# MarinerQ/npf_GWwaveform

Measured on AMD Instinct MI355X. Metric: waveform target-points/sec (train step), higher is better.
Workload: dtype f32 (every contraction of the step: fp32 operands as three exact bf16 terms, six v_mfma_f32_16x16x32_bf16 per product group, f32 accumulation -- f32 results, DESIGN.md 3.1 / 3.2; the 1-4-wide first / last layers: f32 FMAs); 1 GPU; BASELINE config 2: AttnCNP scaledot, r=256, 4-layer xy-encoder/decoder, 256 context / 1024 target points, 256 tasks per GPU (256 global), fp32 train step (fwd+loss+bwd+allreduce+Adam); tasks_per_gpu=256, global_tasks=256, context_points=256, target_points=1024, r_dim=256, n_params=799588, parallelism=dp1, hip_graph=True

## Files before the change

include/npf_hip.h:

```cpp
#ifndef NPF_HIP_H
#define NPF_HIP_H

#include <stdint.h>

#ifdef __cplusplus
extern "C" {
#endif

#define NPF_OK 0
#define NPF_EINVAL (-1)
#define NPF_ELAUNCH (-2)

#define NPF_MAX_OPS 40
#define NPF_MAX_FEATURES 512

enum npf_opcode {
  NPF_OP_END = 0,
  NPF_OP_LOAD_PT = 1,
  NPF_OP_STORE_PT = 2,
  NPF_OP_LOAD_ROWS = 3,
  NPF_OP_STORE_ROWS = 4,
  NPF_OP_LINEAR = 5,
  NPF_OP_SOFTMAX = 6,
  NPF_OP_ADD_PT = 7,
// ... 120 lines not shown
int npf_unpack_pt(const float *pt, int32_t n_tasks, int32_t pts_per_task, int32_t F_valid, float *rows,
                  void *stream);
int npf_transpose(const float *src, int32_t rows, int32_t cols, float *dst, void *stream);
int npf_split_heads(const float *src, int32_t n_tasks, int32_t pts_per_task, int32_t F, int32_t n_heads, float *dst,
                    void *stream);
int npf_merge_heads(const float *src, int32_t n_tasks, int32_t pts_per_task, int32_t F, int32_t n_heads, float *dst,
                    void *stream);

int npf_mha_fwd(const float *q, const float *k, const float *v, int32_t n_tasks, int32_t n_heads, int32_t n_keys,
                int32_t n_queries, int32_t F, float *out, float *lse, void *stream);
int npf_mha_bwd(const float *q, const float *k, const float *v, const float *out, const float *d_out, const float *lse,
                int32_t n_tasks, int32_t n_heads, int32_t n_keys, int32_t n_queries, int32_t F, float *d_q, float *d_k, float *d_v,
                void *stream);

int npf_add_layernorm_fwd(const float *a, const float *b, const float *gamma, const float *beta, float eps, int32_t n_tasks,
                          int32_t pts_per_task, int32_t F, float *y, float *stats, void *stream);
int npf_add_layernorm_bwd(const float *a, const float *b, const float *gamma, const float *stats, const float *dy, int32_t n_tasks,
                          int32_t pts_per_task, int32_t F, float *dx, float *partials, void *stream);

int npf_gather_points(const float *x, const float *y, const int64_t *idx, int32_t n_tasks, int32_t n_points,
                      int32_t n_sel, int32_t x_dim, int32_t y_dim, float *out_x, float *out_y, void *stream);

int npf_cast_bf16_weights(const float *src, int32_t n_rows, int32_t n_cols, int32_t ld, int32_t transposed, void *dst,
                          void *stream);

typedef struct npf_wprep_job {
  const float *src;
  void *dst;
  int32_t n_rows, n_cols, ld, kind;
} npf_wprep_job_t;
#define NPF_MAX_WPREP_JOBS 32
int npf_prepare_weights(const npf_wprep_job_t *jobs, int32_t n_jobs, void *stream);

#define NPF_X6_MAX_LAYERS 8
typedef struct {
  const void *w_img;
  const float *bias;
  const float *mask;
  float *store_in;
  float *store_out;
  const float *addend;
  unsigned long long *store_bits;
  const unsigned long long *mask_bits;
  int32_t relu;
  int32_t reserved;
} npf_x6_layer_t;
int npf_mlp_x6_run(const npf_x6_layer_t *layers, int32_t n_layers, const float *x, float *y, int32_t n_tasks,
                   int32_t tiles_per_task, void *stream);
int npf_mlp_x6_run_rows(const npf_x6_layer_t *layers, int32_t n_layers, const float *x, const float *in_rows, const float *in_w,
                        float *y, const float *out_w, const float *out_b, float *out_rows, int32_t n_tasks,
                        int32_t tiles_per_task, void *stream);

#define NPF_X6_MAX_OPS 12
typedef struct npf_x6_op {
  const float *in_pt;
  const float *in_rows;
  const float *in_w;
  const float *in_b;
  const float *pre_add;
  const float *mask;
  const unsigned long long *mask_bits;
  const float *sbwd_p;
  float *store_in;
  unsigned long long *store_in_bits;
  const void *w_img;
  int64_t w_task_stride;
  const float *bias;
  int64_t bias_task_stride;
  const float *addend;
  float *store_out;
  unsigned long long *store_bits;
  int32_t in_n;
  int32_t in_relu;
  int32_t relu;
  int32_t softmax_n;
  float softmax_scale;
  float sbwd_scale;
  int32_t reserved[2];
} npf_x6_op_t;
#define NPF_X6_IN_RM 1
#define NPF_X6_ADD_RM 2
#define NPF_X6_STORE_IN_F32 4
#define NPF_X6_STORE_OUT_F32 8
#define NPF_X6_DEFAULT_VARIANT 3
int npf_x6_run_ex(const npf_x6_op_t *ops, int32_t n_ops, const float *out_w, const float *out_b, float *out_rows,
                  int32_t n_tasks, int32_t tiles_per_task, int32_t pts_per_task, int32_t per_task, int32_t width,
                  int32_t variant, void *stream);
int npf_x6_run(const npf_x6_op_t *ops, int32_t n_ops, const float *out_w, const float *out_b, float *out_rows,
               int32_t n_tasks, int32_t tiles_per_task, int32_t per_task, int32_t width, void *stream);
int npf_x6_task_images(const float *src, int32_t n_tasks, int32_t pts, int32_t width, void *row_img, void *tr_img, void *stream);

int npf_b16_run(const npf_x6_op_t *ops, int32_t n_ops, const float *out_w, const float *out_b, float *out_rows, int32_t n_tasks,
                int32_t tiles_per_task, int32_t per_task, int32_t width, int32_t variant, void *stream);
int npf_b16_task_images(const float *src, int32_t n_tasks, int32_t pts, int32_t width, void *row_img, void *tr_img, void *stream);

int npf_masked_attn_fwd(const float *q, const float *k, const float *v, const int32_t *n_valid, int32_t n_tasks, int32_t n_keys,
                        int32_t n_queries, int32_t d, float scale, float *out, float *lse, void *stream);
int npf_masked_attn_bwd(const float *q, const float *k, const float *v, const int32_t *n_valid, const float *out, const float *d_out,
                        const float *lse, int32_t n_tasks, int32_t n_keys, int32_t n_queries, int32_t d, float scale, float *d_q,
                        float *d_k, float *d_v, void *stream);
int npf_masked_attn_fwd_nq(const float *q, const float *k, const float *v, const int32_t *n_valid, const int32_t *n_q_valid,
                           int32_t n_tasks, int32_t n_keys, int32_t n_queries, int32_t d, float scale, float *out, float *lse,
                           void *stream);
int npf_masked_attn_bwd_nq(const float *q, const float *k, const float *v, const int32_t *n_valid, const int32_t *n_q_valid,
                           const float *out, const float *d_out, const float *lse, int32_t n_tasks, int32_t n_keys, int32_t n_queries,
                           int32_t d, float scale, float *d_q, float *d_k, float *d_v, void *stream);
int npf_masked_attn_fwd_prefix(const float *q, const float *k_pre, const float *v_pre, const int32_t *n_prefix, const float *k_tail,
                               const float *v_tail, const int32_t *n_tail, const int32_t *n_q_valid, int32_t n_tasks,
                               int32_t n_prefix_tasks, int32_t c_pad, int32_t m_tail, int32_t n_queries, int32_t d, float scale,
                               float *out, void *stream);
int npf_masked_attn_fwd_loo(const float *q, const float *k, const float *v, const int32_t *n_valid, const int32_t *n_q_valid,
                            int32_t n_tasks, int32_t n_keys, int32_t n_queries, int32_t d, float scale, float *out, void *stream);
int npf_masked_mean_fwd(const float *R_pt, const int32_t *n_valid, int32_t n_tasks, int32_t pts_per_task, int32_t F, float *out,
                        void *stream);
int npf_masked_mean_bwd(const float *d_out, const int32_t *n_valid, int32_t n_tasks, int32_t pts_per_task, int32_t F, float *dR_pt,
                        int32_t accumulate, void *stream);
int npf_loo_mean(const float *R_pt, const int32_t *n_valid, int32_t n_tasks, int32_t pts_per_task, int32_t F, float *out,
                 void *stream);

#define NPF_APPEND_MAX_PAIRS 3
typedef struct npf_append_pair {
  const float *src;
  float *dst;
  int32_t F;
  int32_t reserved;
} npf_append_pair_t;
int npf_append_points(const npf_append_pair_t *pairs, int32_t n_pairs, int32_t *n_valid, const int32_t *n_new, int32_t n_tasks,
                      int32_t n_rows, int32_t capacity, void *stream);

int npf_version(void);

#ifdef __cplusplus
}
#endif
#endif
```

npf_gwwaveform_amd/csrc/x6_kernel.hip:

```cpp
#include "x6_args.hpp"


namespace npf {

template <int KF>
struct XpGeom {
  static constexpr int NB = KF / 16;
  static constexpr int KS = KF / 32;
  static constexpr int RowB = KF * 2;
  static constexpr int TermB = 16 * RowB;
  static constexpr int SlabB = 3 * TermB;
  static constexpr int Slots = 3;
  static constexpr int RPP = 1024 / RowB;
  static constexpr int PPT = 16 / RPP;
  static constexpr int NP = 3 * PPT / 4;
  static constexpr int BiasB = 2 * KF * 4;
};

__device__ __forceinline__ void xp_split(const f32x4& lo, const f32x4& hi, xp_u32x4& t0, xp_u32x4& t1, xp_u32x4& t2) {
#ifdef XP_NO_SPLIT
  t0 = __builtin_bit_cast(xp_u32x4, lo);
  t1 = __builtin_bit_cast(xp_u32x4, hi);
  t2 = t0 ^ t1;
  return;
#endif
  const float v[8] = {lo[0], lo[1], lo[2], lo[3], hi[0], hi[1], hi[2], hi[3]};
#pragma unroll
  for (int p = 0; p < 4; ++p) {
    const float a = v[2 * p], b = v[2 * p + 1];
    const unsigned h = xp_cvt_pk(a, b);
    const float ra = a - __builtin_bit_cast(float, h << 16), rb = b - __builtin_bit_cast(float, h & 0xffff0000u);
    const unsigned m = xp_cvt_pk(ra, rb);
    const float la = ra - __builtin_bit_cast(float, m << 16), lb = rb - __builtin_bit_cast(float, m & 0xffff0000u);
    t0[p] = h;
    t1[p] = m;
    t2[p] = xp_cvt_pk(la, lb);
  }
}

template <int KF, int NPG, int NW, int LA = 2>
__global__ __launch_bounds__(NW * 64, (NW == 4 && KF * NPG <= 256) ? 2 : 1) void x6_program_kernel(const XpArgs a) {
  using G = XpGeom<KF>;
  constexpr int NB = G::NB, KS = G::KS;
  constexpr int Slots = LA + 1;
  static_assert(LA >= 2 && LA <= 4 && LA <= NB, "slab look-ahead");
  constexpr int TPW = (NPG == 2 ? 4 : 2) * (NW / 4);
  constexpr int NPW = 3 * G::PPT / NW;
  static_assert(NPG == 1 || NPG == 2, "a wave owns half a tile or a whole one");
  static_assert((NW == 4 || NW == 8) && (3 * G::PPT) % NW == 0 && NPW <= KS, "pieces dealt evenly, one per k-step");
  __shared__ __attribute__((aligned(16))) char smem[Slots * G::SlabB + G::BiasB];
  const int tid = threadIdx.x, lane = tid & 63;
  const int wave = __builtin_amdgcn_readfirstlane(tid >> 6);
  const int p = lane & 15, g = lane >> 4;
  int bid = blockIdx.x;
  if (a.xcd_remap) bid = (bid & 7) * (int)(gridDim.x >> 3) + (bid >> 3);
  const int w_tile = NPG == 2 ? wave : (wave >> 1);
  const int half0 = NPG == 2 ? 0 : (wave & 1);
  int task, t_in;
  bool valid;
  if (a.wgs_per_task > 0) {
    task = bid / a.wgs_per_task;
    t_in = (bid - task * a.wgs_per_task) * TPW + w_tile;
    valid = t_in < a.tiles_per_task;
  } else {
    const long t = (long)bid * TPW + w_tile;
    valid = t < a.total_tiles;
    task = valid ? (int)(t / a.tiles_per_task) : 0;
    t_in = valid ? (int)(t - (long)task * a.tiles_per_task) : 0;
  }
#ifdef XP_NO_STORE
  valid = valid && a.n_ops > 1000;
#endif
  const long tile = valid ? (long)task * a.tiles_per_task + t_in : 0;
  if (a.wgs_per_task == 0) task = 0;
  const size_t tile_off = (size_t)tile * (KF * 32);
  const unsigned lane_b = (unsigned)(((16 * half0 + p) * 4 + g * 128) * 4);
  const size_t bits_off = ((size_t)tile * 2 + half0) * 64;
  const size_t row_off = (size_t)tile * 32 + 16 * half0;
  auto pt32 = [&](const float* base, int pg, int b) -> f32x4* {
    return (f32x4*)((char*)const_cast<float*>(base + tile_off + (size_t)(b * 512 + 64 * pg)) + lane_b);
  };
  auto rm32 = [&](const float* base, int pg, int b) -> const f32x4* {
    int pt = (valid ? t_in : 0) * 32 + 16 * (half0 + pg) + p;
    pt = pt < a.pts_per_task ? pt : a.pts_per_task - 1;
    const size_t tk = valid ? (size_t)(tile / a.tiles_per_task) : 0;
    return (const f32x4*)(base + (tk * a.pts_per_task + (size_t)pt) * KF + 4 * g + 16 * b);
  };

  constexpr int LPR = 64 / G::RPP;
  constexpr int NDL = G::PPT / NW > 0 ? G::PPT / NW : 1;
  unsigned dma_lane[NDL];
#pragma unroll
  for (int n = 0; n < NDL; ++n) {
    const int r0 = G::RPP * ((wave + NW * n) % G::PPT), row = r0 + lane / LPR, pos = lane % LPR;
    dma_lane[n] = (unsigned)((lane / LPR) * G::RowB + ((pos ^ (row & 15)) << 4));
  }
  const int n_slabs = a.n_mm * NB;
  auto dma_piece = [&](const char* img, int rows, char* slot, int n) {
#ifdef XP_NO_DMA
    return;
#endif
    const char* base = img + (size_t)rows * G::RowB;
    asm volatile("" : "+s"(base));
    const int q = wave + NW * n, term = q / G::PPT, r0 = G::RPP * (q % G::PPT);
    xp_dma16(base + (size_t)term * ((size_t)KF * KF * 2) + r0 * G::RowB + dma_lane[n % NDL], slot + term * G::TermB + r0 * G::RowB);
  };
  auto mm_base = [&](int j) { return a.mm_img[j] + (size_t)task * a.mm_stride[j]; };
  auto dma_slab = [&](int S, char* slot) {
    const char* img = mm_base(S / NB);
#pragma unroll
    for (int n = 0; n < NPW; ++n) dma_piece(img, (S % NB) * 16, slot, n);
  };
  const unsigned lds0 = (unsigned)(size_t)(__attribute__((address_space(3))) char*)smem;
  const unsigned lane_row = (unsigned)(p * G::RowB);
  float* bias_lds = (float*)(smem + Slots * G::SlabB);

#pragma unroll
  for (int i = 0; i < LA; ++i)
    if (n_slabs > i) dma_slab(i, smem + i * G::SlabB);
  int slot = 0, S0 = 0, jm = 0;
  f32x4 cur[NPG][NB];
#pragma unroll
  for (int pg = 0; pg < NPG; ++pg)
#pragma unroll
    for (int b = 0; b < NB; ++b) cur[pg][b] = f32x4{0.f, 0.f, 0.f, 0.f};

  for (int l = 0; l < a.n_ops; ++l) {
    const npf_x6_op_t& o = a.op[l];
    const int oflags = o.reserved[0];
#pragma unroll
    for (int pg = 0; pg < NPG; ++pg) {
      if (o.in_pt != nullptr) {
        if (oflags & NPF_X6_IN_RM) {
#pragma unroll
          for (int b = 0; b < NB; ++b) cur[pg][b] = *rm32(o.in_pt, pg, b);
        } else {
#pragma unroll
          for (int b = 0; b < NB; ++b) cur[pg][b] = *pt32(o.in_pt, pg, b);
        }
      }
      if (o.in_rows != nullptr) {
        const f32x4 r = ((const f32x4*)o.in_rows)[row_off + 16 * pg + p];
        const int nb_in = o.in_n >> 4;
#pragma unroll
        for (int b = 0; b < NB; ++b) {
          f32x4 v = {0.f, 0.f, 0.f, 0.f};
          if (b < nb_in) {
            const int f = 16 * b + 4 * g;
            if (o.in_b != nullptr) v = *(const f32x4*)(o.in_b + f);
#pragma unroll
            for (int n = 0; n < 4; ++n) {
              const f32x4 w = *(const f32x4*)(o.in_w + (size_t)n * o.in_n + f);
#pragma unroll
              for (int e = 0; e < 4; ++e) v[e] = fmaf(r[n], w[e], v[e]);
            }
            if (o.in_relu) {
#pragma unroll
              for (int e = 0; e < 4; ++e) v[e] = fmaxf(v[e], 0.f);
            }
          }
          cur[pg][b] = v;
        }
      }
      if (o.pre_add != nullptr) {
#pragma unroll
        for (int b = 0; b < NB; ++b) cur[pg][b] += *pt32(o.pre_add, pg, b);
      }
      if (o.mask != nullptr) {
#pragma unroll
        for (int b = 0; b < NB; ++b) {
          const f32x4 v = *pt32(o.mask, pg, b);
#pragma unroll
          for (int e = 0; e < 4; ++e) cur[pg][b][e] = v[e] > 0.f ? cur[pg][b][e] : 0.f;
        }
      }
      if constexpr (NB <= 16) {
        if (o.mask_bits != nullptr) {
          const unsigned long long w = o.mask_bits[bits_off + 64 * pg + lane];
          const int wl = (int)(unsigned)w, wh = (int)(unsigned)(w >> 32);
#pragma unroll
          for (int b = 0; b < NB; ++b)
#pragma unroll
            for (int e = 0; e < 4; ++e) {
              const int m = __builtin_amdgcn_sbfe(b < 8 ? wl : wh, 4 * (b & 7) + e, 1);
              const float x = cur[pg][b][e];
              cur[pg][b][e] = __int_as_float(__float_as_int(x) & m);
            }
        }
      }
      if constexpr (NB <= 16) if (o.sbwd_p != nullptr) {
        f32x4 P[NB];
        float dot = 0.f;
#pragma unroll
        for (int b = 0; b < NB; ++b) {
          P[b] = *pt32(o.sbwd_p, pg, b);
#pragma unroll
          for (int e = 0; e < 4; ++e) dot = fmaf(cur[pg][b][e], P[b][e], dot);
        }
        dot = xp_sum4(dot);
#pragma unroll
        for (int b = 0; b < NB; ++b)
#pragma unroll
          for (int e = 0; e < 4; ++e) cur[pg][b][e] = o.sbwd_scale * P[b][e] * (cur[pg][b][e] - dot);
      }
      if (o.store_in != nullptr && valid) {
#pragma unroll
        for (int b = 0; b < NB; ++b) __builtin_nontemporal_store(cur[pg][b], pt32(o.store_in, pg, b));
      }
      if constexpr (NB <= 16) {
        if (o.store_in_bits != nullptr && valid) {
          unsigned wlo = 0u, whi = 0u;
#pragma unroll
          for (int b = 0; b < NB; ++b)
#pragma unroll
            for (int e = 0; e < 4; ++e) (b < 8 ? wlo : whi) |= (unsigned)(cur[pg][b][e] > 0.f) << (4 * (b & 7) + e);
          o.store_in_bits[bits_off + 64 * pg + lane] = ((unsigned long long)whi << 32) | wlo;
        }
      }
    }
    if (o.w_img == nullptr) continue;

    for (int i = tid; i < KF; i += NW * 64)
      bias_lds[(jm & 1) * KF + i] = o.bias != nullptr ? o.bias[(size_t)task * o.bias_task_stride + i] : 0.f;
    xp_u32x4 tb[NPG][3][KS];
#pragma unroll
    for (int pg = 0; pg < NPG; ++pg)
#pragma unroll
      for (int st = 0; st < KS; ++st) xp_split(cur[pg][2 * st], cur[pg][2 * st + 1], tb[pg][0][st], tb[pg][1][st], tb[pg][2][st]);
    const bool has_add = o.addend != nullptr;
    if (has_add) {
#pragma unroll
      for (int pg = 0; pg < NPG; ++pg) {
        if (oflags & NPF_X6_ADD_RM) {
#pragma unroll
          for (int b = 0; b < NB; ++b) cur[pg][b] = *rm32(o.addend, pg, b);
        } else {
#pragma unroll
          for (int b = 0; b < NB; ++b) cur[pg][b] = *pt32(o.addend, pg, b);
        }
      }
    }
    const char* const img0 = mm_base(jm);
    const char* const img1 = mm_base(jm + 1 < a.n_mm ? jm + 1 : jm);
    const bool post = NB <= 16 && o.softmax_n > 0;
    const float* const out = (o.store_out != nullptr && valid && !post) ? o.store_out : nullptr;
    const unsigned bias_l = lds0 + Slots * G::SlabB + (jm & 1) * (KF * 4) + g * 16;
    const bool relu = o.relu != 0;
    unsigned pos_lo[NPG], pos_hi[NPG];
#pragma unroll
    for (int pg = 0; pg < NPG; ++pg) pos_lo[pg] = pos_hi[pg] = 0u;
#pragma unroll
    for (int s = 0; s < NB; ++s) {
      const int S = S0 + s;
      {
        const int rem = n_slabs - 1 - S;
#define XP_WAIT(N) asm volatile("s_waitcnt vmcnt(%0) lgkmcnt(0)\n\ts_barrier" ::"n"(N) : "memory")
        if (rem >= LA - 1) XP_WAIT((LA - 1) * NPW);
        else if (LA > 3 && rem == 2) XP_WAIT(2 * NPW);
        else if (LA > 2 && rem == 1) XP_WAIT(NPW);
        else XP_WAIT(0);
#undef XP_WAIT
      }
      const bool more = S + LA < n_slabs;
      char* const nslot = smem + ((slot + LA) % Slots) * G::SlabB;
      const unsigned sl = lds0 + slot * G::SlabB + lane_row;
      f32x4 acc[NPG], sm[NPG];
      xp_u32x4 fr[2][3];
#ifdef XP_NO_FRAG
      acc[0] = f32x4{0.f, 0.f, 0.f, 0.f};
      asm volatile("" : "=v"(fr[0][0]), "=v"(fr[0][1]), "=v"(fr[0][2]), "=v"(fr[1][0]), "=v"(fr[1][1]), "=v"(fr[1][2]));
#else
      asm volatile("ds_read_b128 %0, %4\n\tds_read_b128 %1, %5\n\tds_read_b128 %2, %5 offset:%6\n\tds_read_b128 %3, %5 offset:%7"
                   : "=&v"(acc[0]), "=&v"(fr[0][0]), "=&v"(fr[0][1]), "=&v"(fr[0][2])
                   : "v"(bias_l + 64 * s), "v"(sl + (((0 + g) ^ p) << 4)), "n"(G::TermB), "n"(2 * G::TermB));
#endif
#pragma unroll
      for (int st = 0; st < KS; ++st) {
        const int c = st & 1, n = c ^ 1;
        if (st < NPW && more) {
          asm volatile("s_waitcnt lgkmcnt(0)" ::: "memory");
          dma_piece(s + LA < NB ? img0 : img1, ((s + LA) % NB) * 16, nslot, st);
        }
#ifdef XP_NO_FRAG
        if (false) {
#else
        if (st + 1 < KS) {
#endif
          asm volatile("s_waitcnt lgkmcnt(0)\n\tds_read_b128 %0, %7\n\tds_read_b128 %1, %7 offset:%8\n\tds_read_b128 %2, %7 offset:%9"
                       : "=&v"(fr[n][0]), "=&v"(fr[n][1]), "=&v"(fr[n][2]), "+v"(fr[c][0]), "+v"(fr[c][1]), "+v"(fr[c][2]), "+v"(acc[0])
                       : "v"(sl + (((4 * (st + 1) + g) ^ p) << 4)), "n"(G::TermB), "n"(2 * G::TermB));
        } else {
          asm volatile("s_waitcnt lgkmcnt(0)" : "+v"(fr[c][0]), "+v"(fr[c][1]), "+v"(fr[c][2]), "+v"(acc[0]));
        }
        if (st == 0) {
#pragma unroll
          for (int pg = 0; pg < NPG; ++pg) {
            if (pg > 0) acc[pg] = acc[0];
            sm[pg] = f32x4{0.f, 0.f, 0.f, 0.f};
          }
        }
#ifdef XP_NO_MFMA
#define XPMM(A, B, C, PG) asm volatile("" : "+v"(C[PG]) : "v"(fr[c][A]), "v"(tb[PG][B][st]))
#else
#define XPMM(A, B, C, PG)                                                                                            \
  C[PG] = __builtin_amdgcn_mfma_f32_16x16x32_bf16(__builtin_bit_cast(xp_bf16x8, fr[c][A]),                           \
                                                  __builtin_bit_cast(xp_bf16x8, tb[PG][B][st]), C[PG], 0, 0, 0)
#endif
        if constexpr (NPG == 1) {
          XPMM(2, 0, sm, 0);
          XPMM(0, 0, acc, 0);
          XPMM(0, 2, sm, 0);
          XPMM(1, 0, acc, 0);
          XPMM(1, 1, sm, 0);
          XPMM(0, 1, acc, 0);
        } else {
          XPMM(2, 0, sm, 0);
          XPMM(2, 0, sm, 1);
          XPMM(0, 0, acc, 0);
          XPMM(0, 0, acc, 1);
          XPMM(0, 2, sm, 0);
          XPMM(0, 2, sm, 1);
          XPMM(1, 0, acc, 0);
          XPMM(1, 0, acc, 1);
          XPMM(1, 1, sm, 0);
          XPMM(1, 1, sm, 1);
          XPMM(0, 1, acc, 0);
          XPMM(0, 1, acc, 1);
        }
#undef XPMM
      }
#pragma unroll
      for (int pg = 0; pg < NPG; ++pg) {
        f32x4 r = acc[pg] + sm[pg];
        if (has_add) {
          asm volatile("" ::: "memory");
          r += cur[pg][s];
        }
        if (relu) {
#pragma unroll
          for (int e = 0; e < 4; ++e) {
            float x = r[e];
            asm("v_max_f32 %0, 0, %0" : "+v"(x));
            r[e] = x;
          }
        }
        cur[pg][s] = r;
        if (out != nullptr) __builtin_nontemporal_store(r, pt32(out, pg, s));
        if constexpr (NB <= 16) {
#pragma unroll
          for (int e = 0; e < 4; ++e) (s < 8 ? pos_lo[pg] : pos_hi[pg]) |= (unsigned)(r[e] > 0.f) << (4 * (s & 7) + e);
        }
      }
      slot = (slot + 1) % Slots;
    }
    S0 += NB;
    ++jm;
    if constexpr (NB <= 16) if (post) {
      const float sc = o.softmax_scale;
      const int n_valid = o.softmax_n;
#pragma unroll
      for (int pg = 0; pg < NPG; ++pg) {
        float mx = -INFINITY;
#pragma unroll
        for (int b = 0; b < NB; ++b)
#pragma unroll
          for (int e = 0; e < 4; ++e) {
            const bool ok = 16 * b + 4 * g + e < n_valid;
            cur[pg][b][e] = ok ? sc * cur[pg][b][e] : -INFINITY;
            mx = fmaxf(mx, cur[pg][b][e]);
          }
        mx = xp_max4(mx);
        float sum = 0.f;
#pragma unroll
        for (int b = 0; b < NB; ++b)
#pragma unroll
          for (int e = 0; e < 4; ++e) {
            cur[pg][b][e] = expf(cur[pg][b][e] - mx);
            sum += cur[pg][b][e];
          }
        sum = xp_sum4(sum);
        const float inv = 1.f / sum;
#pragma unroll
        for (int b = 0; b < NB; ++b)
#pragma unroll
          for (int e = 0; e < 4; ++e) cur[pg][b][e] *= inv;
        if (o.store_out != nullptr && valid) {
#pragma unroll
          for (int b = 0; b < NB; ++b) __builtin_nontemporal_store(cur[pg][b], pt32(o.store_out, pg, b));
        }
      }
    }
    if constexpr (NB <= 16) {
      if (o.store_bits != nullptr && valid) {
#pragma unroll
        for (int pg = 0; pg < NPG; ++pg) o.store_bits[bits_off + 64 * pg + lane] = ((unsigned long long)pos_hi[pg] << 32) | pos_lo[pg];
      }
    }
  }

  if (a.out_rows != nullptr) {
    __syncthreads();
    f32x4* wl = (f32x4*)smem;
    for (int i = tid; i < KF; i += NW * 64) wl[i] = ((const f32x4*)a.out_w)[i];
    __syncthreads();
#pragma unroll
    for (int pg = 0; pg < NPG; ++pg) {
      f32x4 r = {0.f, 0.f, 0.f, 0.f};
#pragma unroll
      for (int b = 0; b < NB; ++b)
#pragma unroll
        for (int n = 0; n < 4; ++n) {
          const f32x4 w = wl[n * (KF / 4) + 4 * b + g];
#pragma unroll
          for (int e = 0; e < 4; ++e) r[n] = fmaf(w[e], cur[pg][b][e], r[n]);
        }
#pragma unroll
      for (int n = 0; n < 4; ++n) {
        r[n] = xp_sum4(r[n]);
        if (a.out_b != nullptr) r[n] += a.out_b[n];
      }
      if (valid && g == 0) ((f32x4*)a.out_rows)[row_off + 16 * pg + p] = r;
    }
  }
}

struct XwGeom {
  static constexpr int KF = 512, NB = 32, NBH = 16, KS = 8;
  static constexpr int RowB = KF * 2, TermB = 16 * RowB, SlabB = 3 * TermB, Slots = 3;
  static constexpr int NP = 6;
  static constexpr int BiasB = 2 * KF * 4, XB = 2 * 4 * 1024;
};

__global__ __launch_bounds__(512) void x6_wide512_kernel(const XpArgs a) {
  using G = XwGeom;
  constexpr int KF = G::KF, NB = G::NB, NBH = G::NBH, KS = G::KS;
  __shared__ __attribute__((aligned(16))) char smem[G::Slots * G::SlabB + G::BiasB + G::XB];
  const int tid = threadIdx.x, lane = tid & 63;
  const int wave = __builtin_amdgcn_readfirstlane(tid >> 6);
  const int pg = wave >> 1, kh = wave & 1;
  const int p = lane & 15, g = lane >> 4;
  const long t_flat = (long)blockIdx.x * 2 + (pg >> 1);
  const int half = pg & 1;
  const bool valid = t_flat < a.total_tiles;
  const long tile = valid ? t_flat : 0;
  const int t_in = (int)(tile % a.tiles_per_task);
  const size_t tk = (size_t)(tile / a.tiles_per_task);
  const size_t tile_off = (size_t)tile * (KF * 32);
  const unsigned lane_b = (unsigned)(((16 * half + p) * 4 + g * 128) * 4);
  const size_t row_off = (size_t)tile * 32 + 16 * half;
  auto pt32 = [&](const float* base, int b) -> f32x4* {
    return (f32x4*)((char*)const_cast<float*>(base + tile_off + (size_t)((16 * kh + b) * 512)) + lane_b);
  };
  auto rm32 = [&](const float* base, int b) -> const f32x4* {
    int pt = t_in * 32 + 16 * half + p;
    pt = pt < a.pts_per_task ? pt : a.pts_per_task - 1;
    return (const f32x4*)(base + (tk * a.pts_per_task + (size_t)pt) * KF + 256 * kh + 4 * g + 16 * b);
  };
  unsigned dma_lane[2];
#pragma unroll
  for (int n = 0; n < 2; ++n) dma_lane[n] = (unsigned)((lane ^ ((wave + 8 * n) & 15)) << 4);
  const int n_slabs = a.n_mm * NB;
  auto dma_piece = [&](const char* img, int rows, char* slot, int n) {
    const char* base = img + (size_t)rows * G::RowB;
    asm volatile("" : "+s"(base));
    const int q = wave + 8 * n, term = q >> 4, r0 = q & 15;
    xp_dma16(base + (size_t)term * ((size_t)KF * KF * 2) + r0 * G::RowB + dma_lane[n & 1], slot + term * G::TermB + r0 * G::RowB);
  };
  auto dma_slab = [&](int S, char* slot) {
    const char* img = a.mm_img[S / NB];
#pragma unroll
    for (int n = 0; n < G::NP; ++n) dma_piece(img, (S % NB) * 16, slot, n);
  };
  const unsigned lds0 = (unsigned)(size_t)(__attribute__((address_space(3))) char*)smem;
  const unsigned lane_row = (unsigned)(p * G::RowB);
  float* bias_lds = (float*)(smem + G::Slots * G::SlabB);
  const unsigned xb0 = lds0 + G::Slots * G::SlabB + G::BiasB + (unsigned)(pg * 1024 + lane * 16);

  if (n_slabs > 0) dma_slab(0, smem);
  if (n_slabs > 1) dma_slab(1, smem + G::SlabB);
  int slot = 0, S0 = 0, jm = 0;
  f32x4 cur[NBH];
#pragma unroll
  for (int b = 0; b < NBH; ++b) cur[b] = f32x4{0.f, 0.f, 0.f, 0.f};

  for (int l = 0; l < a.n_ops; ++l) {
    const npf_x6_op_t& o = a.op[l];
    const int oflags = o.reserved[0];
    if (o.in_pt != nullptr) {
      if (oflags & NPF_X6_IN_RM) {
#pragma unroll
        for (int b = 0; b < NBH; ++b) cur[b] = *rm32(o.in_pt, b);
      } else {
#pragma unroll
        for (int b = 0; b < NBH; ++b) cur[b] = *pt32(o.in_pt, b);
      }
    }
    if (o.w_img == nullptr) continue;
    for (int i = tid; i < KF; i += 512) bias_lds[(jm & 1) * KF + i] = o.bias != nullptr ? o.bias[i] : 0.f;
    xp_u32x4 tb[3][KS];
#pragma unroll
    for (int st = 0; st < KS; ++st) xp_split(cur[2 * st], cur[2 * st + 1], tb[0][st], tb[1][st], tb[2][st]);
    const bool has_add = o.addend != nullptr;
    if (has_add) {
      if (oflags & NPF_X6_ADD_RM) {
#pragma unroll
        for (int b = 0; b < NBH; ++b) cur[b] = *rm32(o.addend, b);
      } else {
// ... 106 lines not shown
    __syncthreads();
    if (kh == 0) {
      const f32x4 x = *xb;
#pragma unroll
      for (int n = 0; n < 4; ++n) r[n] += x[n] + (a.out_b != nullptr ? a.out_b[n] : 0.f);
      if (valid && g == 0) ((f32x4*)a.out_rows)[row_off + p] = r;
    }
  }
}

template <int KF, int NT>
__global__ __launch_bounds__(256) void x6_task_images_kernel(const float* __restrict__ src, int tiles_per_task, int pts,
                                                             unsigned short* __restrict__ row_img,
                                                             unsigned short* __restrict__ tr_img) {
  constexpr int TS = KF / 32;
  __shared__ f32x4 tile_s[(KF / 4) * 33];
  const int task = blockIdx.x / TS, ts = blockIdx.x % TS, tid = threadIdx.x;
  const bool have = ts < tiles_per_task;
  if (have) {
    const f32x4* t = (const f32x4*)(src + ((size_t)task * tiles_per_task + ts) * (KF * 32));
    for (int i = tid; i < (KF / 4) * 32; i += 256) {
      const int f4 = i >> 5, pt = i & 31;
      f32x4 v = t[i];
      if (ts * 32 + pt >= pts) v = f32x4{0.f, 0.f, 0.f, 0.f};
      tile_s[f4 * 33 + pt] = v;
    }
  }
  __syncthreads();
  const size_t img = (size_t)KF * KF;
  auto split3 = [](float x, unsigned short& h0, unsigned short& h1, unsigned short& h2) {
    const unsigned a = xp_cvt_pk(x, 0.f) & 0xffffu;
    const float r1 = x - __builtin_bit_cast(float, a << 16);
    const unsigned b = xp_cvt_pk(r1, 0.f) & 0xffffu;
    const float r2 = r1 - __builtin_bit_cast(float, b << 16);
    h0 = (unsigned short)a;
    h1 = (unsigned short)b;
    h2 = (unsigned short)(xp_cvt_pk(r2, 0.f) & 0xffffu);
  };
  if (row_img != nullptr) {
    for (int i = tid; i < 32 * (KF / 8); i += 256) {
      const int pt = i / (KF / 8), ch = i % (KF / 8), st = ch >> 2, gq = ch & 3;
      unsigned short h[3][8];
      if (have) {
        const f32x4 lo = tile_s[(8 * st + gq) * 33 + pt], hi = tile_s[(8 * st + 4 + gq) * 33 + pt];
#pragma unroll
        for (int e = 0; e < 4; ++e) {
          split3(lo[e], h[0][e], h[1][e], h[2][e]);
          split3(hi[e], h[0][4 + e], h[1][4 + e], h[2][4 + e]);
        }
      } else {
#pragma unroll
        for (int q = 0; q < 3; ++q)
#pragma unroll
          for (int e = 0; e < 8; ++e) h[q][e] = 0;
      }
      unsigned short* d = row_img + (size_t)task * NT * img + (size_t)(ts * 32 + pt) * KF + ch * 8;
#pragma unroll
      for (int q = 0; q < NT; ++q) *(uint4*)(d + q * img) = *(const uint4*)h[q];
    }
  }
  if (tr_img != nullptr) {
    for (int i = tid; i < KF * 4; i += 256) {
      const int f = i >> 2, gq = i & 3;
      unsigned short h[3][8];
#pragma unroll
      for (int e = 0; e < 8; ++e) {
        const int pt = (e < 4) ? 4 * gq + e : 16 + 4 * gq + (e - 4);
        const float x = have ? tile_s[(f >> 2) * 33 + pt][f & 3] : 0.f;
        split3(x, h[0][e], h[1][e], h[2][e]);
      }
      unsigned short* d = tr_img + (size_t)task * NT * img + (size_t)f * KF + ts * 32 + gq * 8;
#pragma unroll
      for (int q = 0; q < NT; ++q) *(uint4*)(d + q * img) = *(const uint4*)h[q];
    }
  }
}

}

extern "C" int npf_x6_run_ex(const npf_x6_op_t* ops, int32_t n_ops, const float* out_w, const float* out_b, float* out_rows,
                             int32_t n_tasks, int32_t tiles_per_task, int32_t pts_per_task, int32_t per_task, int32_t width,
                             int32_t variant, void* stream) {
  if (width != 128 && width != 256 && width != 512) return NPF_EINVAL;
  if (variant < 0 || variant > 3 || (variant >= 2 && width == 128) || (variant == 3 && width != 256)) return NPF_EINVAL;
  npf::XpArgs a;
  const int rc = npf::xp_fill_args(ops, n_ops, out_w, out_b, out_rows, n_tasks, tiles_per_task, pts_per_task, per_task, width,
                                   NPF_X6_IN_RM | NPF_X6_ADD_RM, 256, a);
  if (rc != NPF_OK) return rc;
  const int var = width == 256 ? (variant == 0 ? NPF_X6_DEFAULT_VARIANT : variant) : 1;
  const int npg = var == 2 ? 2 : 1;
  const int tpw = var == 1 ? 2 : 4;
  a.wgs_per_task = per_task ? (tiles_per_task + tpw - 1) / tpw : 0;
  const int n_wg = per_task ? n_tasks * a.wgs_per_task : (a.total_tiles + tpw - 1) / tpw;
  a.xcd_remap = (per_task && (n_wg % 8) == 0 && a.wgs_per_task > 1) ? 1 : 0;
  const dim3 grid(n_wg), block(256);
  if (width == 512 && !per_task && variant != 1) {
    bool plain = true;
    for (int l = 0; l < n_ops; ++l) {
      const npf_x6_op_t& o = ops[l];
      if (o.in_rows || o.pre_add || o.mask || o.store_in) plain = false;
    }
    if (plain) {
      hipLaunchKernelGGL(npf::x6_wide512_kernel, dim3((a.total_tiles + 1) / 2), dim3(512), 0, (hipStream_t)stream, a);
      NPF_CHECK_LAUNCH();
      return NPF_OK;
    }
  }
  if (width == 512) hipLaunchKernelGGL((npf::x6_program_kernel<512, 1, 4>), grid, block, 0, (hipStream_t)stream, a);
  else if (width == 128) hipLaunchKernelGGL((npf::x6_program_kernel<128, 1, 4>), grid, block, 0, (hipStream_t)stream, a);
  else if (var == 2) hipLaunchKernelGGL((npf::x6_program_kernel<256, 2, 4>), grid, block, 0, (hipStream_t)stream, a);
  else if (var == 3) hipLaunchKernelGGL((npf::x6_program_kernel<256, 1, 8, 2>), grid, dim3(512), 0, (hipStream_t)stream, a);
  else hipLaunchKernelGGL((npf::x6_program_kernel<256, 1, 4>), grid, block, 0, (hipStream_t)stream, a);
  NPF_CHECK_LAUNCH();
  return NPF_OK;
}

extern "C" int npf_x6_run(const npf_x6_op_t* ops, int32_t n_ops, const float* out_w, const float* out_b, float* out_rows,
                          int32_t n_tasks, int32_t tiles_per_task, int32_t per_task, int32_t width, void* stream) {
  return npf_x6_run_ex(ops, n_ops, out_w, out_b, out_rows, n_tasks, tiles_per_task, tiles_per_task * 32, per_task, width, 0,
                       stream);
}

static int xp_task_images(const float* src, int32_t n_tasks, int32_t pts, int32_t width, void* row_img, void* tr_img, bool one_term,
                          void* stream) {
  if (!src || n_tasks <= 0 || pts <= 0 || pts > width || (width != 128 && width != 256)) return NPF_EINVAL;
  if (!row_img && !tr_img) return NPF_EINVAL;
  if ((((uintptr_t)src) | ((uintptr_t)row_img) | ((uintptr_t)tr_img)) & 15) return NPF_EINVAL;
  const int tiles = (pts + 31) / 32;
  const dim3 grid(n_tasks * (width / 32)), block(256);
  unsigned short *ri = (unsigned short*)row_img, *ti = (unsigned short*)tr_img;
  hipStream_t st = (hipStream_t)stream;
  if (width == 256 && !one_term) hipLaunchKernelGGL((npf::x6_task_images_kernel<256, 3>), grid, block, 0, st, src, tiles, pts, ri, ti);
  else if (width == 256) hipLaunchKernelGGL((npf::x6_task_images_kernel<256, 1>), grid, block, 0, st, src, tiles, pts, ri, ti);
  else if (!one_term) hipLaunchKernelGGL((npf::x6_task_images_kernel<128, 3>), grid, block, 0, st, src, tiles, pts, ri, ti);
  else hipLaunchKernelGGL((npf::x6_task_images_kernel<128, 1>), grid, block, 0, st, src, tiles, pts, ri, ti);
  NPF_CHECK_LAUNCH();
  return NPF_OK;
}

extern "C" int npf_x6_task_images(const float* src, int32_t n_tasks, int32_t pts, int32_t width, void* row_img, void* tr_img,
                                  void* stream) {
  return xp_task_images(src, n_tasks, pts, width, row_img, tr_img, false, stream);
}

extern "C" int npf_b16_task_images(const float* src, int32_t n_tasks, int32_t pts, int32_t width, void* row_img, void* tr_img,
                                   void* stream) {
  return xp_task_images(src, n_tasks, pts, width, row_img, tr_img, true, stream);
}
```

npf_gwwaveform_amd/x6.py:

```python
from __future__ import annotations

import ctypes as C
import math
import os
from typing import List, Optional, Sequence

import torch

from . import _lib as L
from . import chain as CH
from . import functional as FN

ENABLED = os.environ.get("NPF_NO_X6_FUSED", "0") != "1"
WIDTH = 256
VARIANT = int(os.environ.get("NPF_X6_VARIANT", "0"))
B16_ENABLED = os.environ.get("NPF_NO_B16_FUSED", "0") != "1"
B16_VARIANT = int(os.environ.get("NPF_B16_VARIANT", "0"))


class Program:

    def __init__(self, n_tasks: int, tiles: int, per_task: bool, width: int = WIDTH, pts: Optional[int] = None,
                 bf16: bool = False):
        self.n_tasks, self.tiles, self.per_task, self.width = n_tasks, tiles, per_task, width
        self.bf16 = bf16
        self.pts = tiles * 32 if pts is None else pts
        self.ops: List[dict] = []
        self.tail = None
        self.tag = ""

    def op(self, **kw) -> "Program":
        self.ops.append(kw)
        return self

    @staticmethod
    def _ptr(t, what):
        if t is None:
            return None
        if not t.is_cuda or not t.is_contiguous():
            raise RuntimeError(f"x6 program operand {what} must be a contiguous device tensor")
        return t.data_ptr()

    def _pt_ok(self, t, what, p16=False):
        want = (self.n_tasks, self.tiles, self.width // 8, 32, 8) if p16 else (self.n_tasks, self.tiles, self.width // 4, 32, 4)
        dt = torch.bfloat16 if p16 else torch.float32
        if t is not None and (tuple(t.shape) != want or t.dtype != dt):
            raise ValueError(f"x6 program operand {what}: {'PT16' if p16 else 'PT32'} tensor {tuple(t.shape)} {t.dtype}, "
                             f"expected {want} {dt}")

    def launch(self) -> None:
        if len(self.ops) > L.NPF_X6_MAX_OPS:
            raise RuntimeError(f"x6 program longer than NPF_X6_MAX_OPS={L.NPF_X6_MAX_OPS}")
        arr = (L.NpfX6Op * len(self.ops))()
        F, pts = self.width, self.n_tasks * self.tiles * 32
        flops = 0
        nbytes = 0
        for j, o in enumerate(self.ops):
            flags = 0
            for k in ("in_pt", "pre_add", "mask", "sbwd_p", "store_in", "addend", "store_out"):
                t = o.get(k)
                if t is not None and o.get(k + "_rm"):
                    if k not in ("in_pt", "addend") or tuple(t.shape) != (self.n_tasks, self.pts, F) or t.dtype != torch.float32:
                        raise ValueError(f"x6 program operand {k}: row-major tensor {tuple(t.shape)} {t.dtype}")
                    if self.bf16:
                        raise ValueError("b16 programs take no row-major operands")
                    flags |= L.X6_IN_RM if k == "in_pt" else L.X6_ADD_RM
                else:
                    p16 = self.bf16 and (k == "sbwd_p" or (k in ("store_in", "store_out") and not o.get(k + "_f32")))
                    if self.bf16 and k in ("store_in", "store_out") and o.get(k + "_f32") and t is not None:
                        flags |= L.X6_STORE_IN_F32 if k == "store_in" else L.X6_STORE_OUT_F32
                    if self.bf16 and k == "mask" and t is not None:
                        raise ValueError("b16 programs take ReLU masks as bits")
                    self._pt_ok(t, k, p16)
                setattr(arr[j], k, self._ptr(t, k))
                nbytes += pts * F * (t.element_size() if t is not None else 0)
            arr[j].reserved[0] = flags
            for k in ("mask_bits", "store_in_bits", "store_bits"):
                t = o.get(k)
                if t is not None and (tuple(t.shape) != (self.n_tasks, self.tiles, 2, 64) or t.dtype != torch.int64):
                    raise ValueError(f"x6 program operand {k}: bits tensor {tuple(t.shape)} {t.dtype}")
                setattr(arr[j], k, self._ptr(t, k))
                nbytes += pts * F // 8 if t is not None else 0
            if o.get("in_rows") is not None:
                rows, w, b = o["in_rows"], o["in_w"], o.get("in_b")
                n = w.shape[1]
                if tuple(rows.shape) != (self.n_tasks, self.tiles * 32, 4) or w.shape[0] != 4 or n % 16 or n > F:
                    raise ValueError(f"x6 rows prologue: rows {tuple(rows.shape)}, matrix {tuple(w.shape)}")
                if b is not None and tuple(b.shape) != (n,):
                    raise ValueError("x6 rows prologue: bias shape")
                arr[j].in_rows, arr[j].in_w, arr[j].in_b = L.ptr(rows), L.ptr(w), L.ptr(b)
                arr[j].in_n, arr[j].in_relu = n, int(bool(o.get("in_relu", False)))
                flops += 2 * 4 * n * pts
                nbytes += pts * 16
            img = o.get("img")
            if img is not None:
                per_task = bool(o.get("img_per_task", False))
                terms = (1,) if self.bf16 else (3,)
                want = ((self.n_tasks,) if per_task else ()) + (() if self.bf16 else (3,)) + (F, F)
                if tuple(img.shape) != want or img.dtype != torch.bfloat16 or not img.is_contiguous():
                    raise ValueError(f"x6 program weight image {tuple(img.shape)} {img.dtype}, expected {want} bfloat16")
                arr[j].w_img = img.data_ptr()
                arr[j].w_task_stride = terms[0] * F * F * 2 if per_task else 0
                bias = o.get("bias")
                if bias is not None:
                    bpt = bool(o.get("bias_per_task", False))
                    if tuple(bias.shape) != ((self.n_tasks, F) if bpt else (F,)):
                        raise ValueError(f"x6 program bias {tuple(bias.shape)}")
                    arr[j].bias = L.ptr(bias)
                    arr[j].bias_task_stride = F if bpt else 0
                arr[j].relu = int(bool(o.get("relu", False)))
                arr[j].softmax_n = int(o.get("softmax_n", 0))
                arr[j].softmax_scale = float(o.get("softmax_scale", 1.0))
                flops += 2 * o.get("true_k", F) * o.get("true_n", F) * pts
                nbytes += terms[0] * 2 * F * F * (self.n_tasks if per_task else 1)
            elif any(o.get(k) is not None for k in ("bias", "addend", "store_out", "store_bits")) or o.get("relu") or o.get("softmax_n"):
                raise ValueError("x6 program: an op without a multiply has no output side")
            arr[j].sbwd_scale = float(o.get("sbwd_scale", 1.0))
        tail = self.tail
        if tail is not None:
            flops += 2 * 4 * F * pts
            nbytes += pts * 16
        if CH.PROFILE is not None:
            ev0, ev1 = torch.cuda.Event(enable_timing=True), torch.cuda.Event(enable_timing=True)
            ev0.record()
        tw, tb, tr = (L.ptr(tail[0]) if tail else None, L.ptr(tail[1]) if (tail and tail[1] is not None) else None,
                      L.ptr(tail[2]) if tail else None)
        if self.bf16:
            if self.pts != self.tiles * 32:
                raise ValueError("b16 programs run on whole tiles")
            L.check(L.load().npf_b16_run(arr, len(self.ops), tw, tb, tr, self.n_tasks, self.tiles, int(self.per_task), F,
                                         B16_VARIANT, L.stream_ptr()), "npf_b16_run")
        else:
            L.check(L.load().npf_x6_run_ex(arr, len(self.ops), tw, tb, tr, self.n_tasks, self.tiles, self.pts, int(self.per_task), F,
                                           VARIANT if F in (256, 512) else 0, L.stream_ptr()), "npf_x6_run_ex")
        if CH.PROFILE is not None:
            ev1.record()
            CH.PROFILE.append(("b16_program_kernel" if self.bf16 else "x6_program_kernel", flops, ev0, ev1, nbytes, self.tag))
        if CH.TRACE is not None:
            CH.TRACE.append(("prog", self))


def task_images(pt: torch.Tensor, pts: int, row: bool = True, tr: bool = True, width: int = WIDTH, bf16: bool = False):
    n_tasks = pt.shape[0]
    if tuple(pt.shape) != (n_tasks, CH.tiles_of(pts), width // 4, 32, 4) or pts > width:
        raise ValueError(f"task_images: PT32 tensor {tuple(pt.shape)} for {pts} points x {width} features")
    shape = (n_tasks, width, width) if bf16 else (n_tasks, 3, width, width)
    mk = lambda: torch.empty(shape, dtype=torch.bfloat16, device=pt.device)
    ri, ti = (mk() if row else None), (mk() if tr else None)
    if CH.PROFILE is not None:
        ev0, ev1 = torch.cuda.Event(enable_timing=True), torch.cuda.Event(enable_timing=True)
        ev0.record()
    fn = L.load().npf_b16_task_images if bf16 else L.load().npf_x6_task_images
    L.check(fn(L.ptr(pt.detach().contiguous()), n_tasks, pts, width, ri.data_ptr() if row else None,
               ti.data_ptr() if tr else None, L.stream_ptr()), "npf_x6_task_images")
    if CH.PROFILE is not None:
        ev1.record()
        CH.PROFILE.append(("x6_task_images_kernel", 0, ev0, ev1,
                           pt.numel() * 4 + (int(row) + int(tr)) * n_tasks * (1 if bf16 else 3) * width * width * 2))
    return ri, ti


def _weight_images(Ws: Sequence[torch.Tensor], kinds: Sequence[int], width: int = WIDTH, bf16: bool = False) -> List[List[torch.Tensor]]:
    if bf16:
        n = len(Ws)
        buf = torch.empty((len(kinds), n, width, width), dtype=torch.bfloat16, device=Ws[0].device)
        CH.prepare_weights([(Ws[i].detach(), kind) for kind in kinds for i in range(n)],
                           dsts=[buf[k, i] for k in range(len(kinds)) for i in range(n)])
        return [[buf[k, i] for i in range(n)] for k in range(len(kinds))]
    from .mlp_x6 import _three_term_images

    return _three_term_images(Ws, kinds, width)


def _r16(t: Optional[torch.Tensor]) -> Optional[torch.Tensor]:
    return None if t is None else t.to(torch.bfloat16).to(torch.float32)


def _bits(n_tasks, tiles, dev):
    return torch.empty((n_tasks, tiles, 2, 64), dtype=torch.int64, device=dev)


_ZEROS = {}


def _zeros(shape, device) -> torch.Tensor:
    key = (tuple(shape), str(device))
    z = _ZEROS.get(key)
    if z is None:
        z = torch.zeros(shape, dtype=torch.float32, device=device)
        if not (z.is_cuda and torch.cuda.is_current_stream_capturing()):
            _ZEROS[key] = z
    return z


def _pad_rows4(X: torch.Tensor) -> torch.Tensor:
    d = X.shape[-1]
    if d == 4:
        return X.contiguous()
    return torch.cat((X, _zeros((*X.shape[:-1], 4 - d), X.device)), dim=-1)


def _first_layer_matrix(W: torch.Tensor, n_out: int) -> torch.Tensor:
    n, d = W.shape
    Wt = W.detach().t()
    if n < n_out:
        Wt = torch.cat((Wt, _zeros((d, n_out - n), W.device)), dim=1)
    if d < 4:
        Wt = torch.cat((Wt, _zeros((4 - d, n_out), W.device)), dim=0)
    return Wt.contiguous()


def decode_rows_usable(mod, x1: torch.Tensor, x2: torch.Tensor) -> bool:
    from .architectures import MLP

    if not (ENABLED and CH.COMPUTE_DTYPE == "fp32" and mod.is_sum_merge and isinstance(mod.flat_module, MLP)):
        return False
    F = x1.shape[-1]
# ... 870 lines not shown
```

Baseline: 42.79 million target-points/s.

## Stream weight slabs in 32-row units with deeper look-ahead in x6 kernel

Adds an RU template parameter so each pipeline stage loads two 16-row slabs per barrier, which halves the number of s_barrier/waitcnt syncs per image. Look-ahead goes to four blocks (two units), and the next block's bias and fragments are prefetched across the block boundary. This becomes the new default width-256 variant (8 waves), and a width-128 variant 4 is available behind an env switch. The cost is a larger LDS ring, which may reduce occupancy, plus more register pressure from the extra accumulator. Optional timestamp instrumentation is added behind NPF_STAMPS.

Result: faster. 43.51 million target-points/s, median of 6 (+1.7%).

```diff
diff --git a/include/npf_hip.h b/include/npf_hip.h
--- a/include/npf_hip.h
+++ b/include/npf_hip.h
@@ -226,7 +226,7 @@
 #define NPF_X6_ADD_RM 2
 #define NPF_X6_STORE_IN_F32 4
 #define NPF_X6_STORE_OUT_F32 8
-#define NPF_X6_DEFAULT_VARIANT 3
+#define NPF_X6_DEFAULT_VARIANT 4
 int npf_x6_run_ex(const npf_x6_op_t *ops, int32_t n_ops, const float *out_w, const float *out_b, float *out_rows,
                   int32_t n_tasks, int32_t tiles_per_task, int32_t pts_per_task, int32_t per_task, int32_t width,
                   int32_t variant, void *stream);
diff --git a/npf_gwwaveform_amd/csrc/x6_kernel.hip b/npf_gwwaveform_amd/csrc/x6_kernel.hip
--- a/npf_gwwaveform_amd/csrc/x6_kernel.hip
+++ b/npf_gwwaveform_amd/csrc/x6_kernel.hip
@@ -2,6 +2,20 @@
 
 
 namespace npf {
+
+#ifdef NPF_STAMPS
+__device__ unsigned long long g_stamps_x6[16];
+__device__ __forceinline__ unsigned long long xp_stamp() {
+  unsigned long long t;
+  __builtin_amdgcn_sched_barrier(0);
+  asm volatile("s_memtime %0\n\ts_waitcnt lgkmcnt(0)" : "=s"(t)::"memory");
+  __builtin_amdgcn_sched_barrier(0);
+  return t;
+}
+#define XP_STAMP(i) { const unsigned long long t__ = xp_stamp(); st_sum[i] += t__ - st_last; st_last = t__; }
+#else
+#define XP_STAMP(i)
+#endif
 
 template <int KF>
 struct XpGeom {
@@ -38,17 +52,24 @@
   }
 }
 
-template <int KF, int NPG, int NW, int LA = 2>
+template <int KF, int NPG, int NW, int LA = 2, int RU = 16>
 __global__ __launch_bounds__(NW * 64, (NW == 4 && KF * NPG <= 256) ? 2 : 1) void x6_program_kernel(const XpArgs a) {
   using G = XpGeom<KF>;
   constexpr int NB = G::NB, KS = G::KS;
-  constexpr int Slots = LA + 1;
-  static_assert(LA >= 2 && LA <= 4 && LA <= NB, "slab look-ahead");
+  constexpr int UB = RU / 16;
+  constexpr int NU = NB / UB;
+  constexpr int LAU = LA / UB;
+  constexpr int Slots = LAU + 1;
+  constexpr int UnitB = UB * G::SlabB;
+  static_assert((RU == 16 || RU == 32) && NB % UB == 0 && LA % UB == 0, "a unit is one or two 16-row blocks of one image");
+  static_assert(LAU >= 2 && LAU <= 4 && LAU <= NU, "unit look-ahead");
   constexpr int TPW = (NPG == 2 ? 4 : 2) * (NW / 4);
-  constexpr int NPW = 3 * G::PPT / NW;
+  constexpr int NPB = 3 * G::PPT / NW;
+  constexpr int NPW = UB * NPB;
   static_assert(NPG == 1 || NPG == 2, "a wave owns half a tile or a whole one");
-  static_assert((NW == 4 || NW == 8) && (3 * G::PPT) % NW == 0 && NPW <= KS, "pieces dealt evenly, one per k-step");
-  __shared__ __attribute__((aligned(16))) char smem[Slots * G::SlabB + G::BiasB];
+  static_assert((NW == 4 || NW == 8) && (3 * G::PPT) % NW == 0 && NPW <= UB * KS, "pieces dealt evenly, one per k-step of a unit");
+  static_assert(Slots * UnitB + G::BiasB <= 160 * 1024, "the ring and the bias rows fit the CU's LDS");
+  __shared__ __attribute__((aligned(16))) char smem[Slots * UnitB + G::BiasB];
   const int tid = threadIdx.x, lane = tid & 63;
   const int wave = __builtin_amdgcn_readfirstlane(tid >> 6);
   const int p = lane & 15, g = lane >> 4;
@@ -95,7 +116,7 @@
     const int r0 = G::RPP * ((wave + NW * n) % G::PPT), row = r0 + lane / LPR, pos = lane % LPR;
     dma_lane[n] = (unsigned)((lane / LPR) * G::RowB + ((pos ^ (row & 15)) << 4));
   }
-  const int n_slabs = a.n_mm * NB;
+  const int n_slabs = a.n_mm * NU;
   auto dma_piece = [&](const char* img, int rows, char* slot, int n) {
 #ifdef XP_NO_DMA
     return;
@@ -105,19 +126,23 @@
     const int q = wave + NW * n, term = q / G::PPT, r0 = G::RPP * (q % G::PPT);
     xp_dma16(base + (size_t)term * ((size_t)KF * KF * 2) + r0 * G::RowB + dma_lane[n % NDL], slot + term * G::TermB + r0 * G::RowB);
   };
+  auto dma_unit_piece = [&](const char* img, int rows, char* slot, int n) {
+    if constexpr (UB == 1) dma_piece(img, rows, slot, n);
+    else dma_piece(img, rows + 16 * (n / NPB), slot + (n / NPB) * G::SlabB, n % NPB);
+  };
   auto mm_base = [&](int j) { return a.mm_img[j] + (size_t)task * a.mm_stride[j]; };
   auto dma_slab = [&](int S, char* slot) {
-    const char* img = mm_base(S / NB);
-#pragma unroll
-    for (int n = 0; n < NPW; ++n) dma_piece(img, (S % NB) * 16, slot, n);
+    const char* img = mm_base(S / NU);
+#pragma unroll
+    for (int n = 0; n < NPW; ++n) dma_unit_piece(img, (S % NU) * RU, slot, n);
   };
   const unsigned lds0 = (unsigned)(size_t)(__attribute__((address_space(3))) char*)smem;
   const unsigned lane_row = (unsigned)(p * G::RowB);
-  float* bias_lds = (float*)(smem + Slots * G::SlabB);
-
-#pragma unroll
-  for (int i = 0; i < LA; ++i)
-    if (n_slabs > i) dma_slab(i, smem + i * G::SlabB);
+  float* bias_lds = (float*)(smem + Slots * UnitB);
+
+#pragma unroll
+  for (int i = 0; i < LAU; ++i)
+    if (n_slabs > i) dma_slab(i, smem + i * UnitB);
   int slot = 0, S0 = 0, jm = 0;
   f32x4 cur[NPG][NB];
 #pragma unroll
@@ -125,6 +150,12 @@
 #pragma unroll
     for (int b = 0; b < NB; ++b) cur[pg][b] = f32x4{0.f, 0.f, 0.f, 0.f};
 
+#ifdef NPF_STAMPS
+  unsigned long long st_sum[5] = {0, 0, 0, 0, 0};
+  unsigned long long st_last = xp_stamp();
+  const unsigned long long st_first = st_last;
+  unsigned st_syncs = 0;
+#endif
   for (int l = 0; l < a.n_ops; ++l) {
     const npf_x6_op_t& o = a.op[l];
     const int oflags = o.reserved[0];
@@ -244,42 +275,53 @@
     const char* const img1 = mm_base(jm + 1 < a.n_mm ? jm + 1 : jm);
     const bool post = NB <= 16 && o.softmax_n > 0;
     const float* const out = (o.store_out != nullptr && valid && !post) ? o.store_out : nullptr;
-    const unsigned bias_l = lds0 + Slots * G::SlabB + (jm & 1) * (KF * 4) + g * 16;
+    const unsigned bias_l = lds0 + Slots * UnitB + (jm & 1) * (KF * 4) + g * 16;
     const bool relu = o.relu != 0;
     unsigned pos_lo[NPG], pos_hi[NPG];
 #pragma unroll
     for (int pg = 0; pg < NPG; ++pg) pos_lo[pg] = pos_hi[pg] = 0u;
-#pragma unroll
-    for (int s = 0; s < NB; ++s) {
-      const int S = S0 + s;
+    XP_STAMP(0)
+#pragma unroll
+    for (int u = 0; u < NU; ++u) {
+      const int S = S0 + u;
       {
         const int rem = n_slabs - 1 - S;
 #define XP_WAIT(N) asm volatile("s_waitcnt vmcnt(%0) lgkmcnt(0)\n\ts_barrier" ::"n"(N) : "memory")
-        if (rem >= LA - 1) XP_WAIT((LA - 1) * NPW);
-        else if (LA > 3 && rem == 2) XP_WAIT(2 * NPW);
-        else if (LA > 2 && rem == 1) XP_WAIT(NPW);
+        if (rem >= LAU - 1) XP_WAIT((LAU - 1) * NPW);
+        else if (LAU > 3 && rem == 2) XP_WAIT(2 * NPW);
+        else if (LAU > 2 && rem == 1) XP_WAIT(NPW);
         else XP_WAIT(0);
 #undef XP_WAIT
       }
-      const bool more = S + LA < n_slabs;
-      char* const nslot = smem + ((slot + LA) % Slots) * G::SlabB;
-      const unsigned sl = lds0 + slot * G::SlabB + lane_row;
+#ifdef NPF_STAMPS
+      ++st_syncs;
+#endif
+      XP_STAMP(1)
+      const bool more = S + LAU < n_slabs;
+      char* const nslot = smem + ((slot + LAU) % Slots) * UnitB;
+      const unsigned sl = lds0 + slot * UnitB + lane_row;
       f32x4 acc[NPG], sm[NPG];
+      f32x4 accn;
       xp_u32x4 fr[2][3];
 #ifdef XP_NO_FRAG
-      acc[0] = f32x4{0.f, 0.f, 0.f, 0.f};
+      acc[0] = accn = f32x4{0.f, 0.f, 0.f, 0.f};
       asm volatile("" : "=v"(fr[0][0]), "=v"(fr[0][1]), "=v"(fr[0][2]), "=v"(fr[1][0]), "=v"(fr[1][1]), "=v"(fr[1][2]));
 #else
       asm volatile("ds_read_b128 %0, %4\n\tds_read_b128 %1, %5\n\tds_read_b128 %2, %5 offset:%6\n\tds_read_b128 %3, %5 offset:%7"
                    : "=&v"(acc[0]), "=&v"(fr[0][0]), "=&v"(fr[0][1]), "=&v"(fr[0][2])
-                   : "v"(bias_l + 64 * s), "v"(sl + (((0 + g) ^ p) << 4)), "n"(G::TermB), "n"(2 * G::TermB));
-#endif
+                   : "v"(bias_l + 64 * (u * UB)), "v"(sl + (((0 + g) ^ p) << 4)), "n"(G::TermB), "n"(2 * G::TermB));
+#endif
+#pragma unroll
+      for (int j = 0; j < UB; ++j) {
+      const int s = u * UB + j;
+      const unsigned slj = sl + j * G::SlabB;
 #pragma unroll
       for (int st = 0; st < KS; ++st) {
         const int c = st & 1, n = c ^ 1;
-        if (st < NPW && more) {
+        const int ust = j * KS + st;
+        if (ust < NPW && more) {
           asm volatile("s_waitcnt lgkmcnt(0)" ::: "memory");
-          dma_piece(s + LA < NB ? img0 : img1, ((s + LA) % NB) * 16, nslot, st);
+          dma_unit_piece(u + LAU < NU ? img0 : img1, ((u + LAU) % NU) * RU, nslot, ust);
         }
 #ifdef XP_NO_FRAG
         if (false) {
@@ -288,7 +330,16 @@
 #endif
           asm volatile("s_waitcnt lgkmcnt(0)\n\tds_read_b128 %0, %7\n\tds_read_b128 %1, %7 offset:%8\n\tds_read_b128 %2, %7 offset:%9"
                        : "=&v"(fr[n][0]), "=&v"(fr[n][1]), "=&v"(fr[n][2]), "+v"(fr[c][0]), "+v"(fr[c][1]), "+v"(fr[c][2]), "+v"(acc[0])
-                       : "v"(sl + (((4 * (st + 1) + g) ^ p) << 4)), "n"(G::TermB), "n"(2 * G::TermB));
+                       : "v"(slj + (((4 * (st + 1) + g) ^ p) << 4)), "n"(G::TermB), "n"(2 * G::TermB));
+#ifndef XP_NO_FRAG
+        } else if (j + 1 < UB) {
+          static_assert((KS & 1) == 0, "the next block's first fragment lands in fr[0]");
+          asm volatile("s_waitcnt lgkmcnt(0)\n\tds_read_b128 %0, %8\n\tds_read_b128 %1, %9\n\tds_read_b128 %2, %9 offset:%10\n\t"
+                       "ds_read_b128 %3, %9 offset:%11"
+                       : "=&v"(accn), "=&v"(fr[n][0]), "=&v"(fr[n][1]), "=&v"(fr[n][2]), "+v"(fr[c][0]), "+v"(fr[c][1]), "+v"(fr[c][2]),
+                         "+v"(acc[0])
+                       : "v"(bias_l + 64 * (s + 1)), "v"(slj + G::SlabB + (((0 + g) ^ p) << 4)), "n"(G::TermB), "n"(2 * G::TermB));
+#endif
         } else {
           asm volatile("s_waitcnt lgkmcnt(0)" : "+v"(fr[c][0]), "+v"(fr[c][1]), "+v"(fr[c][2]), "+v"(acc[0]));
         }
@@ -298,6 +349,9 @@
             if (pg > 0) acc[pg] = acc[0];
             sm[pg] = f32x4{0.f, 0.f, 0.f, 0.f};
           }
+#ifdef NPF_STAMPS
+          if (j == 0) XP_STAMP(2)
+#endif
         }
 #ifdef XP_NO_MFMA
 #define XPMM(A, B, C, PG) asm volatile("" : "+v"(C[PG]) : "v"(fr[c][A]), "v"(tb[PG][B][st]))
@@ -329,6 +383,8 @@
         }
 #undef XPMM
       }
+      XP_STAMP(3)
+      if (j + 1 < UB) asm volatile("s_waitcnt lgkmcnt(0)" ::: "memory");
 #pragma unroll
       for (int pg = 0; pg < NPG; ++pg) {
         f32x4 r = acc[pg] + sm[pg];
@@ -351,9 +407,15 @@
           for (int e = 0; e < 4; ++e) (s < 8 ? pos_lo[pg] : pos_hi[pg]) |= (unsigned)(r[e] > 0.f) << (4 * (s & 7) + e);
         }
       }
+      if (j + 1 < UB) {
+        asm volatile("" ::: "memory");
+        acc[0] = accn;
+      }
+      XP_STAMP(4)
+      }
       slot = (slot + 1) % Slots;
     }
-    S0 += NB;
+    S0 += NU;
     ++jm;
     if constexpr (NB <= 16) if (post) {
       const float sc = o.softmax_scale;
@@ -422,7 +484,23 @@
       if (valid && g == 0) ((f32x4*)a.out_rows)[row_off + 16 * pg + p] = r;
     }
   }
-}
+#ifdef NPF_STAMPS
+  XP_STAMP(0)
+  if (blockIdx.x == 0 && tid == 0) {
+    for (int i = 0; i < 5; ++i) g_stamps_x6[i] = st_sum[i];
+    g_stamps_x6[8] = st_last - st_first;
+    g_stamps_x6[9] = st_syncs;
+  }
+#endif
+}
+
+#ifdef NPF_STAMPS
+}
+extern "C" int npf_debug_stamps_x6(unsigned long long* host16) {
+  return hipMemcpyFromSymbol(host16, HIP_SYMBOL(npf::g_stamps_x6), 16 * sizeof(unsigned long long)) == hipSuccess ? 0 : -1;
+}
+namespace npf {
+#endif
 
 struct XwGeom {
   static constexpr int KF = 512, NB = 32, NBH = 16, KS = 8;
@@ -695,14 +773,14 @@
                              int32_t n_tasks, int32_t tiles_per_task, int32_t pts_per_task, int32_t per_task, int32_t width,
                              int32_t variant, void* stream) {
   if (width != 128 && width != 256 && width != 512) return NPF_EINVAL;
-  if (variant < 0 || variant > 3 || (variant >= 2 && width == 128) || (variant == 3 && width != 256)) return NPF_EINVAL;
+  if (variant < 0 || variant > 4 || ((variant == 2 || variant == 3) && width == 128) || (variant >= 3 && width == 512)) return NPF_EINVAL;
   npf::XpArgs a;
   const int rc = npf::xp_fill_args(ops, n_ops, out_w, out_b, out_rows, n_tasks, tiles_per_task, pts_per_task, per_task, width,
                                    NPF_X6_IN_RM | NPF_X6_ADD_RM, 256, a);
   if (rc != NPF_OK) return rc;
-  const int var = width == 256 ? (variant == 0 ? NPF_X6_DEFAULT_VARIANT : variant) : 1;
+  const int var = width == 256 ? (variant == 0 ? NPF_X6_DEFAULT_VARIANT : variant) : (width == 128 && variant == 4 ? 4 : 1);
   const int npg = var == 2 ? 2 : 1;
-  const int tpw = var == 1 ? 2 : 4;
+  const int tpw = (var == 1 || width == 128) ? 2 : 4;
   a.wgs_per_task = per_task ? (tiles_per_task + tpw - 1) / tpw : 0;
   const int n_wg = per_task ? n_tasks * a.wgs_per_task : (a.total_tiles + tpw - 1) / tpw;
   a.xcd_remap = (per_task && (n_wg % 8) == 0 && a.wgs_per_task > 1) ? 1 : 0;
@@ -720,8 +798,10 @@
     }
   }
   if (width == 512) hipLaunchKernelGGL((npf::x6_program_kernel<512, 1, 4>), grid, block, 0, (hipStream_t)stream, a);
+  else if (width == 128 && var == 4) hipLaunchKernelGGL((npf::x6_program_kernel<128, 1, 4, 4, 32>), grid, block, 0, (hipStream_t)stream, a);
   else if (width == 128) hipLaunchKernelGGL((npf::x6_program_kernel<128, 1, 4>), grid, block, 0, (hipStream_t)stream, a);
   else if (var == 2) hipLaunchKernelGGL((npf::x6_program_kernel<256, 2, 4>), grid, block, 0, (hipStream_t)stream, a);
+  else if (var == 4) hipLaunchKernelGGL((npf::x6_program_kernel<256, 1, 8, 4, 32>), grid, dim3(512), 0, (hipStream_t)stream, a);
   else if (var == 3) hipLaunchKernelGGL((npf::x6_program_kernel<256, 1, 8, 2>), grid, dim3(512), 0, (hipStream_t)stream, a);
   else hipLaunchKernelGGL((npf::x6_program_kernel<256, 1, 4>), grid, block, 0, (hipStream_t)stream, a);
   NPF_CHECK_LAUNCH();
diff --git a/npf_gwwaveform_amd/x6.py b/npf_gwwaveform_amd/x6.py
--- a/npf_gwwaveform_amd/x6.py
+++ b/npf_gwwaveform_amd/x6.py
@@ -14,6 +14,12 @@
 ENABLED = os.environ.get("NPF_NO_X6_FUSED", "0") != "1"
 WIDTH = 256
 VARIANT = int(os.environ.get("NPF_X6_VARIANT", "0"))
+
+
+def _variant_for(width: int) -> int:
+    if VARIANT == 4:
+        return 4 if width in (128, 256) else 0
+    return VARIANT if width in (256, 512) else 0
 B16_ENABLED = os.environ.get("NPF_NO_B16_FUSED", "0") != "1"
 B16_VARIANT = int(os.environ.get("NPF_B16_VARIANT", "0"))
 
@@ -132,7 +138,7 @@
                                          B16_VARIANT, L.stream_ptr()), "npf_b16_run")
         else:
             L.check(L.load().npf_x6_run_ex(arr, len(self.ops), tw, tb, tr, self.n_tasks, self.tiles, self.pts, int(self.per_task), F,
-                                           VARIANT if F in (256, 512) else 0, L.stream_ptr()), "npf_x6_run_ex")
+                                           _variant_for(F), L.stream_ptr()), "npf_x6_run_ex")
         if CH.PROFILE is not None:
             ev1.record()
             CH.PROFILE.append(("b16_program_kernel" if self.bf16 else "x6_program_kernel", flops, ev0, ev1, nbytes, self.tag))
```
